# AdaptiveCity/deepdish

Measured on AMD Instinct MI355X. Metric: end-to-end frames/sec (detect+encode+track) at 640x480, higher is better.
Workload: dtype i8 (reference: uint8); encoder f16; 1 GPU; SSD-MobileNet-v1 uint8-quantised (300x300) + MARS-64x32x3 + deep_sort on synthetic 640x480 BGR frames, ~20 synthetic detections/frame (BASELINE.json configs[1]); streams_per_gpu=3072, worker_threads_per_gpu=2, parallelism=independent streams, 3072 per GPU in 2 worker groups, weights=seeded synthetic (seed 1234)

## Files before the change

### deepdish_amd/csrc/cost_dev.h

```cpp
#pragma once
#include <hip/hip_runtime.h>

namespace costdev {

typedef float f32x4 __attribute__((ext_vector_type(4)));

__device__ __forceinline__ double iou_tlwh(const double *a, const double *b) {
    const double ax2 = a[0] + a[2], ay2 = a[1] + a[3];
    const double bx2 = b[0] + b[2], by2 = b[1] + b[3];
    const double tlx = fmax(a[0], b[0]), tly = fmax(a[1], b[1]);
    const double brx = fmin(ax2, bx2), bry = fmin(ay2, by2);
    const double w = fmax(0.0, brx - tlx), h = fmax(0.0, bry - tly);
    const double inter = w * h;
    const double area_a = a[2] * a[3];
    const double area_b = b[2] * b[3];
    return inter / (area_a + area_b - inter);
}

constexpr int GAL_CH_SHIFT = 5, GAL_CH = 1 << GAL_CH_SHIFT;
constexpr int GAL_ARENA_SHIFT = 12, GAL_ARENA_CHUNKS = 1 << GAL_ARENA_SHIFT;

__device__ __forceinline__ float *gal_row(float *const *arenas, int chunk, int off) {
    return arenas[chunk >> GAL_ARENA_SHIFT] + ((size_t)(chunk & (GAL_ARENA_CHUNKS - 1)) * GAL_CH + off) * 128;
}

struct FlatRows {
    const float *base;
    __device__ __forceinline__ const float *row(int r) const { return base + (size_t)r * 128; }
};

struct ChunkRows {
    float *const *arenas;
    const int *tab;
    __device__ __forceinline__ const float *row(int r) const { return gal_row(arenas, tab[r >> GAL_CH_SHIFT], r & (GAL_CH - 1)); }
};

template <class Rows>
__device__ __forceinline__ float nn_max_dot(const Rows rows, int count,
                                            const float *__restrict__ feats, int d0, int n_d, int lane) {
    const int c = lane & 15, q = lane >> 4;
    const int dd = min(d0 + c, n_d - 1);
    f32x4 b[8];
    const float *fp = feats + (size_t)dd * 128 + 4 * q;
#pragma unroll
    for (int s = 0; s < 8; ++s) b[s] = *reinterpret_cast<const f32x4 *>(fp + 16 * s);
    float best = -__builtin_inff();
    for (int g = 0; g < count; g += 16) {
        const int r = min(g + c, count - 1);
        const float *ap = rows.row(r) + 4 * q;
        f32x4 acc = {0.f, 0.f, 0.f, 0.f};
#pragma unroll
        for (int s = 0; s < 8; ++s) {
            const f32x4 a = *reinterpret_cast<const f32x4 *>(ap + 16 * s);
#pragma unroll
            for (int j = 0; j < 4; ++j) acc = __builtin_amdgcn_mfma_f32_16x16x4f32(a[j], b[s][j], acc, 0, 0, 0);
        }
        best = fmaxf(best, fmaxf(fmaxf(acc[0], acc[1]), fmaxf(acc[2], acc[3])));
    }
    best = fmaxf(best, __shfl_xor(best, 16, 64));
    best = fmaxf(best, __shfl_xor(best, 32, 64));
    return best;
}

template <class Rows>
__device__ __forceinline__ float nn_min_sqdist(const Rows rows, int count,
                                               const float *__restrict__ feats, int d0, int n_d, int lane) {
    const int c = lane & 15, q = lane >> 4;
    const int dd = min(d0 + c, n_d - 1);
    f32x4 b[8];
    const float *fp = feats + (size_t)dd * 128 + 4 * q;
    f32x4 b2 = {0.f, 0.f, 0.f, 0.f};
#pragma unroll
    for (int s = 0; s < 8; ++s) {
        b[s] = *reinterpret_cast<const f32x4 *>(fp + 16 * s);
        b2 += b[s] * b[s];
    }
    float qn = (b2[0] + b2[1]) + (b2[2] + b2[3]);
    qn += __shfl_xor(qn, 16, 64);
    qn += __shfl_xor(qn, 32, 64);
    float best = __builtin_inff();
    for (int g = 0; g < count; g += 16) {
        const int r = min(g + c, count - 1);
        const float *ap = rows.row(r) + 4 * q;
        f32x4 acc = {0.f, 0.f, 0.f, 0.f}, a2 = {0.f, 0.f, 0.f, 0.f};
#pragma unroll
        for (int s = 0; s < 8; ++s) {
            const f32x4 a = *reinterpret_cast<const f32x4 *>(ap + 16 * s);
            a2 += a * a;
#pragma unroll
            for (int j = 0; j < 4; ++j) acc = __builtin_amdgcn_mfma_f32_16x16x4f32(a[j], b[s][j], acc, 0, 0, 0);
        }
        float rn = (a2[0] + a2[1]) + (a2[2] + a2[3]);
        rn += __shfl_xor(rn, 16, 64);
        rn += __shfl_xor(rn, 32, 64);
#pragma unroll
        for (int j = 0; j < 4; ++j) {
            const float gn = __shfl(rn, 4 * q + j, 64);
            best = fminf(best, fmaxf(0.f, (-2.f * acc[j] + gn) + qn));
        }
    }
    best = fminf(best, __shfl_xor(best, 16, 64));
    best = fminf(best, __shfl_xor(best, 32, 64));
    return best;
}

}
```

### deepdish_amd/csrc/tracker.hip

```cpp
#include <algorithm>
#include <atomic>
#include <numeric>
#include "common.h"
#include "hostpool.h"
#include "kalman_dev.h"
#include "cost_dev.h"

namespace {
using namespace kfdev;
using namespace costdev;

constexpr double GATE_4DOF = 9.4877;
constexpr double INFTY_COST = 1e5;
enum { TENTATIVE = 1, CONFIRMED = 2, DELETED = 3 };
enum { METRIC_COSINE = 0, METRIC_EUCLIDEAN = 1 };
enum { ASSOC_HOST = 0, ASSOC_DEVICE = 1 };

__device__ __forceinline__ void tlwh_to_xyah(const double *b, double z[4]) {
    z[0] = b[0] + b[2] / 2;
    z[1] = b[1] + b[3] / 2;
    z[2] = b[2] / b[3];
    z[3] = b[3];
}

template <int Metric>
__global__ __launch_bounds__(256) void tracker_assoc_k(
    const double *__restrict__ means, const double *__restrict__ covs, float *const *__restrict__ arenas,
    const int *__restrict__ tab, int tab_stride, const int *__restrict__ row_slot, const int *__restrict__ row_state,
    const int *__restrict__ row_tsu, const int *__restrict__ row_det_off, const int *__restrict__ row_ndet,
    const int *__restrict__ row_cost_off, const int *__restrict__ row_iou_delta, const int *__restrict__ row_gcount,
    const double *__restrict__ det_tlwh, const float *__restrict__ feats_n, double *__restrict__ cost) {
    const int row = blockIdx.x;
    const int wave = threadIdx.x >> 6, lane = threadIdx.x & 63;
    const int n_det = row_ndet[row];
    const int d0 = blockIdx.y * 64 + wave * 16;
    if (d0 >= n_det) return;
    const int slot = row_slot[row];
    const int det_off = row_det_off[row];
    const bool confirmed = row_state[row] == CONFIRMED;
    float best = 0.f;
    if (confirmed) {
        if constexpr (Metric == METRIC_EUCLIDEAN)
            best = nn_min_sqdist(ChunkRows{arenas, tab + (size_t)slot * tab_stride}, row_gcount[row],
                                 feats_n + (size_t)det_off * 128, d0, n_det, lane);
        else
            best = nn_max_dot(ChunkRows{arenas, tab + (size_t)slot * tab_stride}, row_gcount[row],
                              feats_n + (size_t)det_off * 128, d0, n_det, lane);
    }
    const int d = d0 + (lane & 15);
    if ((lane >> 4) != 0 || d >= n_det) return;
    const double *m = means + (size_t)slot * 8;
    const double *b = det_tlwh + (size_t)(det_off + d) * 4;
    const size_t o = (size_t)row_cost_off[row] + d;
    if (confirmed) {
        double S[16], z[4];
        innovation_cov(covs + (size_t)slot * 64, m[3], S);
        const Chol4 c = chol4(S);
        tlwh_to_xyah(b, z);
        const double mm[4] = {m[0], m[1], m[2], m[3]};
        const double d2 = maha2(c, mm, z, 0);
        if constexpr (Metric == METRIC_EUCLIDEAN) cost[o] = d2 > GATE_4DOF ? INFTY_COST : (double)best;
        else cost[o] = d2 > GATE_4DOF ? INFTY_COST : (double)(1.0f - best);
    }
    double ci = INFTY_COST;
    if (row_tsu[row] <= 1) {
        double t[4];
        t[3] = m[3];
        t[2] = m[2] * m[3];
        t[0] = m[0] - t[2] / 2;
        t[1] = m[1] - t[3] / 2;
        ci = 1.0 - iou_tlwh(t, b);
    }
    cost[o + row_iou_delta[row]] = ci;
}

__global__ __launch_bounds__(256) void tracker_apply_k(
    double *__restrict__ means, double *__restrict__ covs, float *const *__restrict__ arenas,
    const int *__restrict__ pair_slot, const int *__restrict__ pair_det, const int *__restrict__ pair_row, int n_upd,
    int n_new, const double *__restrict__ det_tlwh, const float *__restrict__ feats_n) {
    const int w = (blockIdx.x * blockDim.x + threadIdx.x) >> 6;
    const int lane = threadIdx.x & 63;
    if (w >= n_upd + n_new) return;
    const int slot = pair_slot[w], det = pair_det[w], grow = pair_row[w];
    double z[4];
    tlwh_to_xyah(det_tlwh + (size_t)det * 4, z);
    double *P = covs + (size_t)slot * 64, *m = means + (size_t)slot * 8;
    if (w < n_upd) update_wave(P, m, z, lane);
    else initiate_wave(P, m, z, lane);
    const float2 f = reinterpret_cast<const float2 *>(feats_n + (size_t)det * 128)[lane];
    reinterpret_cast<float2 *>(gal_row(arenas, grow >> GAL_CH_SHIFT, grow & (GAL_CH - 1)))[lane] = f;
}

__global__ void tab_scatter_k(int *__restrict__ tab, const int *__restrict__ upd, int n) {
    const int i = blockIdx.x * blockDim.x + threadIdx.x;
    if (i < n) tab[upd[2 * i]] = upd[2 * i + 1];
}

struct TrackRec {
    int64_t id;
    int state, tsu, hits, age, slot, last_det;
};

}

constexpr int GAL_MAX_ARENAS = 4096;
struct TrackerPool {
    dd_ctx *ctx = nullptr;
    int slots = 0, refs = 0;
    int metric = 0;
    double *d_means = nullptr, *d_covs = nullptr;
    std::vector<float *> arenas;
    float **d_arenas = nullptr;
    std::vector<int> free_chunks;
    std::vector<std::vector<int>> slot_chunks;
    std::vector<int> slot_total;
    int *d_tab = nullptr, tab_stride = 0;
    std::vector<int> tab_upd;
    int tab_need = 0;
    DevBuf d_tabupd;
    PinBuf h_tabupd;
    DevBuf d_pred, d_in, d_feats_raw, d_feats_n, d_cost, d_pairs, d_gather, d_assoc;
    PinBuf h_pred, h_in, h_cost, h_pairs, h_gather, h_assoc;
    bool pred_inflight = false;
    int assoc = 0;
    bool upd_inflight = false;
    bool dev_decided = false;
    bool cost_on_host = false;
    std::vector<int> assoc_base;
    long long n_dev_updates = 0, n_host_updates = 0, n_fallback_streams = 0;
    long long assoc_d2h_bytes = 0;
    long long n_stream_param_launches = 0;
    std::vector<dd_tracker *> cur;
    std::vector<int> det_off, cost_base;
    int D = 0, R = 0, ng = 0;
    bool have_cost = false;
};

struct dd_tracker {
    TrackerPool *pool = nullptr;
    int slot_base = 0;
    double max_cos = 0.2, max_iou = 0.7;
    int max_age = 30, n_init = 3, budget = 0, tcap = 0;
    std::vector<TrackRec> tracks, deleted;
    std::vector<int> free_slots, pending_free;
    std::vector<double> live_means, dead_means;
    std::vector<int> last_pairs;
    int64_t next_id = 1;
    int ph_n = 0, ph_T = 0, ph_cost_base = -1;
    std::vector<int> m_upd, m_new;
};

namespace {

void min_cost_matching(const double *full, int n_det, double max_distance, const std::vector<int> &rows,
                       const std::vector<int> &dets, std::vector<std::pair<int, int>> &matches,
                       std::vector<int> &un_rows, std::vector<int> &un_dets) {
    un_rows.clear();
    un_dets.clear();
    if (rows.empty() || dets.empty()) {
        un_rows = rows;
        un_dets = dets;
        return;
    }
    const int nr = (int)rows.size(), nc = (int)dets.size();
    std::vector<double> c((size_t)nr * nc);
    for (int r = 0; r < nr; ++r)
        for (int q = 0; q < nc; ++q) {
            const double v = full[(size_t)rows[r] * n_det + dets[q]];
            c[(size_t)r * nc + q] = v > max_distance ? max_distance + 1e-5 : v;
        }
    std::vector<int> ri(std::min(nr, nc)), ci(std::min(nr, nc));
    const int np = ddk::lsap(c.data(), nr, nc, ri.data(), ci.data());
    std::vector<char> row_used(nr, 0), col_used(nc, 0);
    for (int p = 0; p < np; ++p) { row_used[ri[p]] = 1; col_used[ci[p]] = 1; }
    for (int q = 0; q < nc; ++q) if (!col_used[q]) un_dets.push_back(dets[q]);
    for (int r = 0; r < nr; ++r) if (!row_used[r]) un_rows.push_back(rows[r]);
    for (int p = 0; p < np; ++p) {
        if (c[(size_t)ri[p] * nc + ci[p]] > max_distance) {
            un_rows.push_back(rows[ri[p]]);
            un_dets.push_back(dets[ci[p]]);
        } else {
            matches.emplace_back(rows[ri[p]], dets[ci[p]]);
        }
    }
}

int pool_create(dd_ctx *ctx, int slots, int gallery_rows_hint, TrackerPool **out) {
    TrackerPool *p = new TrackerPool();
    p->ctx = ctx; p->slots = slots;
    DD_HIP(hipSetDevice(ctx->device));
    DD_HIP(hipMalloc(&p->d_means, (size_t)slots * 8 * sizeof(double)));
    DD_HIP(hipMalloc(&p->d_covs, (size_t)slots * 64 * sizeof(double)));
    DD_HIP(hipMalloc(&p->d_arenas, (size_t)GAL_MAX_ARENAS * sizeof(float *)));
    DD_HIP(hipMemset(p->d_arenas, 0, (size_t)GAL_MAX_ARENAS * sizeof(float *)));
    p->tab_stride = std::max(1, dd_ceil_div(gallery_rows_hint, GAL_CH));
    DD_HIP(hipMalloc(&p->d_tab, (size_t)slots * p->tab_stride * sizeof(int)));
    DD_HIP(hipMemset(p->d_tab, 0, (size_t)slots * p->tab_stride * sizeof(int)));
    p->slot_chunks.resize(slots);
    p->slot_total.assign(slots, 0);
    *out = p;
    return DD_OK;
}

int pool_add_arena(TrackerPool *p) {
    DD_REQUIRE((int)p->arenas.size() < GAL_MAX_ARENAS, DD_E_CAPACITY, "tracker gallery: %d arenas of 64 MiB exhausted", GAL_MAX_ARENAS);
    float *a = nullptr;
    const hipError_t e = hipMalloc(&a, (size_t)GAL_ARENA_CHUNKS * GAL_CH * 128 * sizeof(float));
    if (e != hipSuccess) {
        (void)hipGetLastError();
        dd_set_error("tracker gallery: device memory exhausted after %zu arenas of 64 MiB (%s); nn_budget bounds a gallery",
                     p->arenas.size(), hipGetErrorString(e));
        return DD_E_CAPACITY;
    }
    const int k = (int)p->arenas.size();
    p->arenas.push_back(a);
    DD_HIP(hipMemcpy(p->d_arenas + k, &a, sizeof(float *), hipMemcpyHostToDevice));
    for (int c = GAL_ARENA_CHUNKS - 1; c >= 0; --c) p->free_chunks.push_back(k * GAL_ARENA_CHUNKS + c);
    return DD_OK;
}

int gallery_place(TrackerPool *p, int slot, int budget, int *row_out) {
    const int total = p->slot_total[slot];
    const int pos = budget > 0 ? total % budget : total;
    const int ci = pos >> GAL_CH_SHIFT;
    std::vector<int> &chs = p->slot_chunks[slot];
    if (ci >= (int)chs.size()) {
        p->tab_need = std::max(p->tab_need, ci + 1);
        if (p->free_chunks.empty()) {
            const int rc = pool_add_arena(p);
            if (rc != DD_OK) return rc;
        }
        const int c = p->free_chunks.back();
        p->free_chunks.pop_back();
        chs.push_back(c);
        p->tab_upd.push_back(slot);
        p->tab_upd.push_back(ci);
        p->tab_upd.push_back(c);
    }
    *row_out = chs[ci] * GAL_CH + (pos & (GAL_CH - 1));
    p->slot_total[slot] = total + 1;
    return DD_OK;
}

inline int gallery_count(const TrackerPool *p, int slot, int budget) {
    const int total = p->slot_total[slot];
    return budget > 0 ? std::min(total, budget) : total;
}

void gallery_free_slot(TrackerPool *p, int slot) {
    for (int c : p->slot_chunks[slot]) p->free_chunks.push_back(c);
    p->slot_chunks[slot].clear();
    p->slot_total[slot] = 0;
}

int gallery_flush(TrackerPool *p, hipStream_t s) {
    if (p->tab_need > p->tab_stride) {
        int stride = p->tab_stride;
        while (p->tab_need > stride) stride *= 2;
        DD_HIP(hipStreamSynchronize(s));
        const size_t n = (size_t)p->slots * stride;
        int *fresh = nullptr;
        DD_HIP(hipMalloc(&fresh, n * sizeof(int)));
        std::vector<int> host(n, 0);
        for (int sl = 0; sl < p->slots; ++sl)
            for (size_t i = 0; i < p->slot_chunks[sl].size(); ++i) host[(size_t)sl * stride + i] = p->slot_chunks[sl][i];
        const hipError_t e = hipMemcpy(fresh, host.data(), n * sizeof(int), hipMemcpyHostToDevice);
        if (e != hipSuccess) { (void)hipFree(fresh); DD_HIP(e); }
        (void)hipFree(p->d_tab);
        p->d_tab = fresh; p->tab_stride = stride;
        p->tab_upd.clear();
        return DD_OK;
    }
    const int n = (int)p->tab_upd.size() / 3;
    if (n == 0) return DD_OK;
    int rc;
    if ((rc = p->h_tabupd.reserve((size_t)n * 2 * sizeof(int))) != DD_OK) return rc;
    if ((rc = p->d_tabupd.reserve((size_t)n * 2 * sizeof(int))) != DD_OK) return rc;
    int *h = p->h_tabupd.as<int>();
    for (int i = 0; i < n; ++i) {
        h[2 * i] = p->tab_upd[3 * i] * p->tab_stride + p->tab_upd[3 * i + 1];
        h[2 * i + 1] = p->tab_upd[3 * i + 2];
    }
    p->tab_upd.clear();
    DD_HIP(hipMemcpyAsync(p->d_tabupd.p, h, (size_t)n * 2 * sizeof(int), hipMemcpyHostToDevice, s));
    hipLaunchKernelGGL(tab_scatter_k, dim3(dd_ceil_div(n, 256)), dim3(256), 0, s, p->d_tab, p->d_tabupd.as<int>(), n);
    DD_LAUNCH_CHECK();
    return DD_OK;
}

void pool_release(TrackerPool *p) {
    if (!p || --p->refs > 0) return;
    (void)hipFree(p->d_means); (void)hipFree(p->d_covs);
    for (float *a : p->arenas) (void)hipFree(a);
    (void)hipFree(p->d_arenas); (void)hipFree(p->d_tab);
    for (DevBuf *b : {&p->d_pred, &p->d_in, &p->d_feats_raw, &p->d_feats_n, &p->d_cost, &p->d_pairs, &p->d_gather, &p->d_tabupd, &p->d_assoc}) b->release();
    for (PinBuf *b : {&p->h_pred, &p->h_in, &p->h_cost, &p->h_pairs, &p->h_gather, &p->h_tabupd, &p->h_assoc}) b->release();
    delete p;
}

dd_tracker *tracker_new(TrackerPool *pool, int slot_base, int tcap, double max_cos, double max_iou, int max_age, int n_init,
                        int budget) {
    dd_tracker *t = new dd_tracker();
    t->pool = pool; pool->refs += 1;
    t->slot_base = slot_base; t->tcap = tcap;
    t->max_cos = max_cos; t->max_iou = max_iou; t->max_age = max_age; t->n_init = n_init;
    t->budget = budget > 0 ? budget : 0;
    t->free_slots.resize(tcap);
    for (int i = 0; i < tcap; ++i) t->free_slots[i] = slot_base + tcap - 1 - i;
    return t;
}

}

namespace ddk {

int tracker_group_create(dd_ctx *ctx, int n, double max_cos, double max_iou, int max_age, int n_init, int budget, int tcap,
                         int gcap, dd_tracker **out) {
    TrackerPool *pool = nullptr;
    int rc = pool_create(ctx, n * tcap, gcap, &pool);
    if (rc != DD_OK) return rc;
    for (int i = 0; i < n; ++i) out[i] = tracker_new(pool, i * tcap, tcap, max_cos, max_iou, max_age, n_init, budget);
    return DD_OK;
}

int tracker_set_params(dd_tracker *t, const double *max_cos, const double *max_iou, const int *max_age, const int *n_init) {
    DD_REQUIRE(t, DD_E_ARG, "tracker_set_params: NULL tracker");
    DD_REQUIRE(!t->pool->upd_inflight, DD_E_STATE, "tracker parameters: an update of the group is in flight");
    if (max_cos) t->max_cos = *max_cos;
    if (max_iou) t->max_iou = *max_iou;
    if (max_age) t->max_age = *max_age;
    if (n_init) t->n_init = *n_init;
    return DD_OK;
}

int tracker_reset(dd_tracker *t) {
    DD_REQUIRE(t, DD_E_ARG, "tracker_reset: NULL tracker");
    TrackerPool *p = t->pool;
    DD_REQUIRE(!p->upd_inflight, DD_E_STATE, "tracker reset: an update of the group is in flight");
    for (int sl : t->pending_free) gallery_free_slot(p, sl);
    for (auto &tr : t->tracks) gallery_free_slot(p, tr.slot);
    t->pending_free.clear(); t->tracks.clear(); t->deleted.clear();
    t->live_means.clear(); t->dead_means.clear(); t->last_pairs.clear(); t->m_upd.clear(); t->m_new.clear();
    t->next_id = 1;
    t->ph_n = t->ph_T = 0; t->ph_cost_base = -1;
    t->free_slots.resize(t->tcap);
    for (int i = 0; i < t->tcap; ++i) t->free_slots[i] = t->slot_base + t->tcap - 1 - i;
    return DD_OK;
}

long long tracker_group_stream_param_launches(const dd_tracker *any) { return any ? any->pool->n_stream_param_launches : 0; }

int tracker_group_set_metric(dd_tracker *any, int metric) {
    DD_REQUIRE(any && (metric == METRIC_COSINE || metric == METRIC_EUCLIDEAN), DD_E_ARG,
               "tracker metric must be 0 (cosine) or 1 (euclidean), got %d", metric);
    TrackerPool *p = any->pool;
    DD_REQUIRE(p->arenas.empty() || p->metric == metric, DD_E_STATE, "tracker metric: the group already holds gallery rows");
    p->metric = metric;
    return DD_OK;
}

int tracker_group_set_association(dd_tracker *any, int where) {
    DD_REQUIRE(any && (where == ASSOC_HOST || where == ASSOC_DEVICE), DD_E_ARG,
               "tracker association must be 0 (host) or 1 (device), got %d", where);
    DD_REQUIRE(!any->pool->upd_inflight, DD_E_STATE, "tracker association: an update of the group is in flight");
    any->pool->assoc = where;
    return DD_OK;
}

int trackers_predict(dd_tracker **ts, int S) {
    if (S <= 0) return DD_OK;
    TrackerPool *p = ts[0]->pool;
    hipStream_t s = p->ctx->stream;
    int n = 0;
    for (int z = 0; z < S; ++z) {
        dd_tracker *t = ts[z];
        for (int sl : t->pending_free) { gallery_free_slot(p, sl); t->free_slots.push_back(sl); }
        t->pending_free.clear();
        n += (int)t->tracks.size();
    }
    if (n == 0) return DD_OK;
    int rc;
    if (p->pred_inflight) DD_HIP(hipStreamSynchronize(s));
    p->pred_inflight = true;
    if ((rc = p->h_pred.reserve((size_t)n * sizeof(int))) != DD_OK) return rc;
    if ((rc = p->d_pred.reserve((size_t)n * sizeof(int))) != DD_OK) return rc;
    int *h = p->h_pred.as<int>();
    int k = 0;
    for (int z = 0; z < S; ++z)
        for (auto &tr : ts[z]->tracks) {
            h[k++] = tr.slot;
            tr.age += 1;
            tr.tsu += 1;
        }
    DD_HIP(hipMemcpyAsync(p->d_pred.p, h, (size_t)n * sizeof(int), hipMemcpyHostToDevice, s));
    return ddk::kf_predict(s, p->d_means, p->d_covs, p->d_pred.as<int>(), n);
}

int trackers_update_begin(dd_tracker **ts, int S, const double *tlwh_host, const float *feats, int feats_on_device,
                          const int *det_off) {
    TrackerPool *p = ts[0]->pool;
    hipStream_t s = p->ctx->stream;
    int rc;
    if ((p->tab_need > p->tab_stride || !p->tab_upd.empty()) && (rc = gallery_flush(p, s)) != DD_OK) return rc;
    p->cur.assign(ts, ts + S);
    p->det_off.assign(det_off, det_off + S + 1);
    p->cost_base.assign(S, 0);
    const int D = det_off[S];
    int R = 0, maxn = 0;
    size_t cost_total = 0;
    for (int z = 0; z < S; ++z) {
        dd_tracker *t = ts[z];
        t->last_pairs.clear();
        for (auto &tr : t->tracks) tr.last_det = -1;
        t->ph_n = det_off[z + 1] - det_off[z];
        t->ph_T = (int)t->tracks.size();
        p->cost_base[z] = (int)cost_total;
        cost_total += (size_t)2 * t->ph_T * t->ph_n;
        R += t->ph_T;
        maxn = std::max(maxn, t->ph_n);
    }
    p->D = D; p->R = R; p->have_cost = false;
    bool use_dev = p->assoc == ASSOC_DEVICE;
    for (int z = 0; z < S && use_dev; ++z) use_dev = ts[z]->ph_T <= DD_ASSOC_DEVICE_MAX && ts[z]->ph_n <= DD_ASSOC_DEVICE_MAX;
    p->dev_decided = use_dev; p->cost_on_host = false;
    p->assoc_base.assign(S, -1);
    long long &n_updates = use_dev ? p->n_dev_updates : p->n_host_updates;
    if (D == 0) {
        n_updates += 1;
        p->upd_inflight = true;
        return DD_OK;
    }
    bool par_differ = false;
    for (int z = 1; z < S && use_dev && !par_differ; ++z)
        par_differ = ts[z]->max_cos != ts[0]->max_cos || ts[z]->max_iou != ts[0]->max_iou || ts[z]->max_age != ts[0]->max_age;
    const size_t off_rows = (size_t)D * 4 * sizeof(double);
    const size_t off_desc = off_rows + (size_t)8 * R * sizeof(int);
    const size_t off_par = (off_desc + (size_t)5 * S * sizeof(int) + 7) / 8 * 8, off_age = off_par + (size_t)2 * S * sizeof(double);
    const size_t in_bytes = !use_dev ? off_desc : par_differ ? off_age + (size_t)S * sizeof(int) : off_desc + (size_t)5 * S * sizeof(int);
    if ((rc = p->h_in.reserve(in_bytes + 64)) != DD_OK) return rc;
    if ((rc = p->d_in.reserve(in_bytes + 64)) != DD_OK) return rc;
    char *h = p->h_in.as<char>();
    memcpy(h, tlwh_host, (size_t)D * 4 * sizeof(double));
    int *hr = reinterpret_cast<int *>(h + off_rows);
    int *h_slot = hr, *h_state = hr + R, *h_tsu = hr + 2 * R, *h_doff = hr + 3 * R, *h_nd = hr + 4 * R, *h_coff = hr + 5 * R,
        *h_idel = hr + 6 * R, *h_gcnt = hr + 7 * R;
    int r = 0;
    for (int z = 0; z < S; ++z) {
        dd_tracker *t = ts[z];
        for (int i = 0; i < t->ph_T; ++i, ++r) {
            h_slot[r] = t->tracks[i].slot;
            h_state[r] = t->tracks[i].state;
            h_tsu[r] = t->tracks[i].tsu;
            h_doff[r] = det_off[z];
            h_nd[r] = t->ph_n;
            h_coff[r] = p->cost_base[z] + i * t->ph_n;
            h_idel[r] = t->ph_T * t->ph_n;
            h_gcnt[r] = gallery_count(p, t->tracks[i].slot, t->budget);
        }
    }
    int n_dec = 0;
    size_t out_ints = 0;
    if (use_dev) {
        int *hd = reinterpret_cast<int *>(h + off_desc);
        double *hpd = reinterpret_cast<double *>(h + off_par);
        int *hpa = reinterpret_cast<int *>(h + off_age);
        int row_base = 0;
        for (int z = 0; z < S; ++z) {
            const dd_tracker *t = ts[z];
            if (t->ph_T > 0 && t->ph_n > 0) {
                if (par_differ) { hpd[2 * n_dec] = t->max_cos; hpd[2 * n_dec + 1] = t->max_iou; hpa[n_dec] = t->max_age; }
                int *e = hd + 5 * n_dec++;
                e[0] = row_base; e[1] = t->ph_T; e[2] = t->ph_n; e[3] = p->cost_base[z]; e[4] = (int)out_ints;
                p->assoc_base[z] = (int)out_ints;
                out_ints += ddk::assoc_out_ints(t->ph_T, t->ph_n);
            }
            row_base += t->ph_T;
        }
    }
    char *d = p->d_in.as<char>();
    DD_HIP(hipMemcpyAsync(d, h, in_bytes, hipMemcpyHostToDevice, s));
    const bool euclid = p->metric == METRIC_EUCLIDEAN;
    if ((rc = p->d_feats_n.reserve((size_t)D * 128 * sizeof(float))) != DD_OK) return rc;
    if (euclid) {
        DD_HIP(hipMemcpyAsync(p->d_feats_n.p, feats, (size_t)D * 128 * sizeof(float),
                              feats_on_device ? hipMemcpyDeviceToDevice : hipMemcpyHostToDevice, s));
    } else {
        const float *raw = feats;
        if (!feats_on_device) {
            if ((rc = p->d_feats_raw.reserve((size_t)D * 128 * sizeof(float))) != DD_OK) return rc;
            DD_HIP(hipMemcpyAsync(p->d_feats_raw.p, feats, (size_t)D * 128 * sizeof(float), hipMemcpyHostToDevice, s));
            raw = p->d_feats_raw.as<float>();
        }
        if ((rc = ddk::normalize_rows(s, raw, p->d_feats_n.as<float>(), D)) != DD_OK) return rc;
    }
    if (R > 0 && cost_total > 0) {
        if ((rc = p->d_cost.reserve(cost_total * sizeof(double))) != DD_OK) return rc;
        if (!use_dev && (rc = p->h_cost.reserve(cost_total * sizeof(double))) != DD_OK) return rc;
        const int *dr = reinterpret_cast<const int *>(d + off_rows);
        hipLaunchKernelGGL(euclid ? tracker_assoc_k<METRIC_EUCLIDEAN> : tracker_assoc_k<METRIC_COSINE>, dim3(R, dd_ceil_div(maxn, 64)),
                           dim3(256), 0, s, p->d_means, p->d_covs,
                           p->d_arenas, p->d_tab, p->tab_stride, dr, dr + R, dr + 2 * R, dr + 3 * R, dr + 4 * R, dr + 5 * R,
                           dr + 6 * R, dr + 7 * R, reinterpret_cast<const double *>(d), p->d_feats_n.as<float>(),
                           p->d_cost.as<double>());
        DD_LAUNCH_CHECK();
        if (use_dev) {
            if ((rc = p->d_assoc.reserve(out_ints * sizeof(int))) != DD_OK) return rc;
            if ((rc = p->h_assoc.reserve(out_ints * sizeof(int))) != DD_OK) return rc;
            if (par_differ) {
                if ((rc = ddk::assoc_match_streams(s, p->d_cost.as<double>(), dr + R, dr + 2 * R, reinterpret_cast<const int *>(d + off_desc), n_dec,
                                                   reinterpret_cast<const double *>(d + off_par), reinterpret_cast<const int *>(d + off_age),
                                                   p->d_assoc.as<int>())) != DD_OK) return rc;
                p->n_stream_param_launches += n_dec > 0;
            } else
            if ((rc = ddk::assoc_match(s, p->d_cost.as<double>(), dr + R, dr + 2 * R, reinterpret_cast<const int *>(d + off_desc), n_dec,
                                       ts[0]->max_cos, ts[0]->max_iou, ts[0]->max_age, p->d_assoc.as<int>())) != DD_OK) return rc;
            DD_HIP(hipMemcpyAsync(p->h_assoc.p, p->d_assoc.p, out_ints * sizeof(int), hipMemcpyDeviceToHost, s));
            p->assoc_d2h_bytes += (long long)(out_ints * sizeof(int));
        } else {
            DD_HIP(hipMemcpyAsync(p->h_cost.p, p->d_cost.p, cost_total * sizeof(double), hipMemcpyDeviceToHost, s));
            p->cost_on_host = true;
            p->assoc_d2h_bytes += (long long)(cost_total * sizeof(double));
        }
        p->have_cost = true;
    }
    n_updates += 1;
    p->upd_inflight = true;
    return DD_OK;
}

namespace {
int match_one_stream(TrackerPool *p, dd_tracker *t, int z) {
    const int n = t->ph_n, T = t->ph_T, doff = p->det_off[z];
    std::vector<int> matches, un_rows_final, un_dets;
    t->m_upd.clear(); t->m_new.clear();
    t->ph_cost_base = (n > 0 && T > 0 && p->have_cost) ? p->cost_base[z] : -1;
    const int *dev = (p->dev_decided && n > 0 && T > 0 && p->assoc_base[z] >= 0) ? p->h_assoc.as<int>() + p->assoc_base[z] : nullptr;
    if (dev && dev[0] == 0) {
        const int *pm = dev + 4, *pr = pm + 2 * std::min(T, n), *pd = pr + T;
        matches.assign(pm, pm + 2 * dev[1]);
        un_rows_final.assign(pr, pr + dev[2]);
        un_dets.assign(pd, pd + dev[3]);
    } else {
        std::vector<int> state(T), tsu(T);
        for (int i = 0; i < T; ++i) { state[i] = t->tracks[i].state; tsu[i] = t->tracks[i].tsu; }
        const double *app = (n > 0 && T > 0) ? p->h_cost.as<double>() + p->cost_base[z] : nullptr;
        ddk::match_decide_host(app, app ? app + (size_t)T * n : nullptr, T, n, state.data(), tsu.data(), t->max_cos, t->max_iou, t->max_age,
                               matches, un_rows_final, un_dets);
    }
    for (size_t k = 0; k + 1 < matches.size(); k += 2) {
        const int row = matches[k], det = matches[k + 1];
        TrackRec &tr = t->tracks[row];
        tr.hits += 1;
        tr.tsu = 0;
        tr.last_det = det;
        if (tr.state == TENTATIVE && tr.hits >= t->n_init) tr.state = CONFIRMED;
        t->m_upd.push_back(tr.slot); t->m_upd.push_back(doff + det);
        t->last_pairs.push_back(row);
        t->last_pairs.push_back(det);
    }
    for (int r : un_rows_final) {
        TrackRec &tr = t->tracks[r];
        if (tr.state == TENTATIVE) tr.state = DELETED;
        else if (tr.tsu > t->max_age) tr.state = DELETED;
    }
    DD_REQUIRE((int)t->free_slots.size() >= (int)un_dets.size(), DD_E_CAPACITY,
               "dd_tracker_update: track capacity %d exhausted", t->tcap);
    for (int dd : un_dets) {
        TrackRec tr;
        tr.id = t->next_id++;
        tr.state = TENTATIVE; tr.tsu = 0; tr.hits = 1; tr.age = 1;
        tr.slot = t->free_slots.back();
        t->free_slots.pop_back();
        tr.last_det = dd;
        t->tracks.push_back(tr);
        t->m_new.push_back(tr.slot); t->m_new.push_back(doff + dd);
    }
    std::vector<TrackRec> live;
    t->deleted.clear();
    for (auto &tr : t->tracks) (tr.state == DELETED ? t->deleted : live).push_back(tr);
    t->tracks.swap(live);
    for (auto &tr : t->deleted) t->pending_free.push_back(tr.slot);
    return DD_OK;
}
}

void match_decide_host(const double *app, const double *iou, int T, int n, const int *state, const int *tsu, double max_cos,
                       double max_iou, int max_age, std::vector<int> &matches_flat, std::vector<int> &un_rows_final, std::vector<int> &un_dets) {
    std::vector<std::pair<int, int>> matches;
    std::vector<int> lvl_rows, tmp_rows, tmp_dets, confirmed, unconfirmed;
    matches_flat.clear(); un_rows_final.clear(); un_dets.clear();
    if (n > 0 && T > 0) {
        for (int i = 0; i < T; ++i) (state[i] == CONFIRMED ? confirmed : unconfirmed).push_back(i);
        un_dets.resize(n);
        std::iota(un_dets.begin(), un_dets.end(), 0);
        for (int level = 0; level < max_age; ++level) {
            if (un_dets.empty()) break;
            lvl_rows.clear();
            for (int k : confirmed) if (tsu[k] == 1 + level) lvl_rows.push_back(k);
            if (lvl_rows.empty()) continue;
            min_cost_matching(app, n, max_cos, lvl_rows, un_dets, matches, tmp_rows, tmp_dets);
            un_dets = tmp_dets;
        }
        std::vector<int> matched_rows, un_a_all;
        for (auto &m : matches) matched_rows.push_back(m.first);
        ddk::pyset_difference_order(confirmed, matched_rows, un_a_all);
        std::vector<int> iou_rows = unconfirmed, un_rows_a;
        for (int k : un_a_all) {
            if (tsu[k] == 1) iou_rows.push_back(k); else un_rows_a.push_back(k);
        }
        std::vector<int> un_rows_b;
        min_cost_matching(iou, n, max_iou, iou_rows, un_dets, matches, un_rows_b, tmp_dets);
        un_dets = tmp_dets;
        un_rows_final = un_rows_a;
        un_rows_final.insert(un_rows_final.end(), un_rows_b.begin(), un_rows_b.end());
    } else {
        un_dets.resize(n);
        std::iota(un_dets.begin(), un_dets.end(), 0);
        for (int i = 0; i < T; ++i) un_rows_final.push_back(i);
    }
    for (auto &m : matches) { matches_flat.push_back(m.first); matches_flat.push_back(m.second); }
}

namespace {
int update_match(dd_tracker **ts, int S) {
    TrackerPool *p = ts[0]->pool;
    hipStream_t s = p->ctx->stream;
    p->pred_inflight = false;
    int rc;
    const int D = p->D;
    if (p->dev_decided && p->have_cost) {
        size_t total = 0;
        for (int z = 0; z < S; ++z) total += (size_t)2 * ts[z]->ph_T * ts[z]->ph_n;
        int n_back = 0;
        for (int z = 0; z < S; ++z) {
            if (p->assoc_base[z] < 0 || p->h_assoc.as<int>()[p->assoc_base[z]] == 0) continue;
            if (n_back++ == 0 && (rc = p->h_cost.reserve(total * sizeof(double))) != DD_OK) return rc;
            const size_t bytes = (size_t)2 * ts[z]->ph_T * ts[z]->ph_n * sizeof(double);
            DD_HIP(hipMemcpyAsync(p->h_cost.as<double>() + p->cost_base[z], p->d_cost.as<double>() + p->cost_base[z], bytes,
                                  hipMemcpyDeviceToHost, s));
            p->assoc_d2h_bytes += (long long)bytes;
        }
        if (n_back) DD_HIP(hipStreamSynchronize(s));
        p->n_fallback_streams += n_back;
    }
    size_t max_pairs = (size_t)p->R + D;
    if ((rc = p->h_pairs.reserve(max_pairs * 3 * sizeof(int) + 64)) != DD_OK) return rc;
    if ((rc = p->d_pairs.reserve(max_pairs * 3 * sizeof(int) + 64)) != DD_OK) return rc;
    std::vector<int> upd_slot, upd_det, upd_row, new_slot, new_det, new_row;
    std::atomic<int> first_err{DD_OK};
    ddk::parallel_for(S, 8, [&](int z0, int z1) {
        for (int z = z0; z < z1; ++z) {
            const int r = match_one_stream(p, ts[z], z);
            if (r != DD_OK) { int ok = DD_OK; first_err.compare_exchange_strong(ok, r); }
        }
    });
    if (first_err.load() != DD_OK) {
        int zbad = -1;
        for (int z = 0; z < S && zbad < 0; ++z) if (ts[z]->free_slots.empty()) zbad = z;
        dd_set_error("dd_tracker_update: track capacity %d exhausted (stream %d of %d in the group); the group's state is no longer consistent: "
                     "recreate it with a larger track_capacity", zbad >= 0 ? ts[zbad]->tcap : ts[0]->tcap, zbad, S);
        return first_err.load();
    }
    for (int z = 0; z < S; ++z) {
        dd_tracker *t = ts[z];
        for (size_t i = 0; i + 1 < t->m_upd.size(); i += 2) {
            int grow = 0;
            if ((rc = gallery_place(p, t->m_upd[i], t->budget, &grow)) != DD_OK) return rc;
            upd_slot.push_back(t->m_upd[i]); upd_det.push_back(t->m_upd[i + 1]); upd_row.push_back(grow);
        }
        for (size_t i = 0; i + 1 < t->m_new.size(); i += 2) {
            int grow = 0;
            if ((rc = gallery_place(p, t->m_new[i], t->budget, &grow)) != DD_OK) return rc;
            new_slot.push_back(t->m_new[i]); new_det.push_back(t->m_new[i + 1]); new_row.push_back(grow);
        }
    }
    const int n_upd = (int)upd_slot.size(), n_new = (int)new_slot.size(), np = n_upd + n_new;
    if (np > 0) {
        int *hp = p->h_pairs.as<int>();
        for (int i = 0; i < n_upd; ++i) { hp[i] = upd_slot[i]; hp[np + i] = upd_det[i]; hp[2 * np + i] = upd_row[i]; }
        for (int i = 0; i < n_new; ++i) { hp[n_upd + i] = new_slot[i]; hp[np + n_upd + i] = new_det[i]; hp[2 * np + n_upd + i] = new_row[i]; }
        int *dp = p->d_pairs.as<int>();
        DD_HIP(hipMemcpyAsync(dp, hp, (size_t)3 * np * sizeof(int), hipMemcpyHostToDevice, s));
        hipLaunchKernelGGL(tracker_apply_k, dim3(dd_ceil_div(np, 4)), dim3(256), 0, s, p->d_means, p->d_covs, p->d_arenas,
                           dp, dp + np, dp + 2 * np, n_upd, n_new, p->d_in.as<double>(), p->d_feats_n.as<float>());
        DD_LAUNCH_CHECK();
    }
    if ((rc = gallery_flush(p, s)) != DD_OK) return rc;
    int ng = 0;
    for (int z = 0; z < S; ++z) ng += (int)(ts[z]->tracks.size() + ts[z]->deleted.size());
    p->ng = ng;
    if (ng > 0) {
        if ((rc = p->h_gather.reserve((size_t)ng * (sizeof(int) + 8 * sizeof(double)))) != DD_OK) return rc;
        if ((rc = p->d_gather.reserve((size_t)ng * (sizeof(int) + 8 * sizeof(double)))) != DD_OK) return rc;
        double *hg = p->h_gather.as<double>();
        int *hs = reinterpret_cast<int *>(hg + (size_t)ng * 8);
        int k = 0;
        for (int z = 0; z < S; ++z) {
            for (auto &tr : ts[z]->tracks) hs[k++] = tr.slot;
            for (auto &tr : ts[z]->deleted) hs[k++] = tr.slot;
        }
        double *dg = p->d_gather.as<double>();
        int *ds = reinterpret_cast<int *>(dg + (size_t)ng * 8);
        DD_HIP(hipMemcpyAsync(ds, hs, (size_t)ng * sizeof(int), hipMemcpyHostToDevice, s));
        if ((rc = ddk::gather_state(s, p->d_means, p->d_covs, ds, ng, dg, nullptr)) != DD_OK) return rc;
        DD_HIP(hipMemcpyAsync(hg, dg, (size_t)ng * 8 * sizeof(double), hipMemcpyDeviceToHost, s));
    }
    return DD_OK;
}
}

int trackers_update_match(dd_tracker **ts, int S) {
    const int rc = update_match(ts, S);
    if (rc != DD_OK) ts[0]->pool->upd_inflight = false;
    return rc;
}

int trackers_update_end(dd_tracker **ts, int S) {
    TrackerPool *p = ts[0]->pool;
    p->upd_inflight = false;
    const double *hg = p->h_gather.as<double>();
    size_t k = 0;
    for (int z = 0; z < S; ++z) {
        dd_tracker *t = ts[z];
        const size_t nl = t->tracks.size(), nd = t->deleted.size();
        t->live_means.assign(hg + k * 8, hg + (k + nl) * 8);
        k += nl;
        t->dead_means.assign(hg + k * 8, hg + (k + nd) * 8);
        k += nd;
    }
    return DD_OK;
}

int tracker_read_host(dd_tracker *t, int which, int64_t *ints6_host, double *means_host) {
    const std::vector<TrackRec> &v = which == 0 ? t->tracks : t->deleted;
    const std::vector<double> &mm = which == 0 ? t->live_means : t->dead_means;
    const int n = (int)v.size();
    if (ints6_host)
        for (int i = 0; i < n; ++i) {
            int64_t *o = ints6_host + (size_t)i * 6;
            o[0] = v[i].id; o[1] = v[i].state; o[2] = v[i].tsu; o[3] = v[i].hits; o[4] = v[i].age; o[5] = v[i].last_det;
        }
    if (means_host && n) {
        DD_REQUIRE(mm.size() == (size_t)n * 8, DD_E_STATE, "dd_tracker_read: means are only mirrored after update()");
        memcpy(means_host, mm.data(), (size_t)n * 8 * sizeof(double));
    }
    return DD_OK;
}


void tracker_pool_view(dd_tracker *t, TrackerPoolView *v) {
    TrackerPool *p = t->pool;
    v->d_arenas = p->d_arenas; v->d_means = p->d_means; v->d_covs = p->d_covs;
    v->arena_shift = GAL_ARENA_SHIFT; v->metric = p->metric; v->budget = t->budget; v->tcap = t->tcap;
    v->max_cos = t->max_cos; v->max_iou = t->max_iou; v->max_age = t->max_age; v->n_init = t->n_init;
    v->upd_inflight = p->upd_inflight;
}

int tracker_export(dd_tracker *t, int64_t *next_id, std::vector<TrackView> &live, std::vector<TrackView> &dead) {
    TrackerPool *p = t->pool;
    DD_REQUIRE(t->live_means.size() == t->tracks.size() * 8 && t->dead_means.size() == t->deleted.size() * 8, DD_E_STATE,
               "snapshot: the tracker's means are not mirrored (between a per-track call and the next update)");
    *next_id = t->next_id;
    for (int which = 0; which < 2; ++which) {
        const std::vector<TrackRec> &v = which == 0 ? t->tracks : t->deleted;
        std::vector<TrackView> &out = which == 0 ? live : dead;
        out.clear();
        for (const TrackRec &tr : v) {
            TrackView w;
            w.id = tr.id; w.state = tr.state; w.tsu = tr.tsu; w.hits = tr.hits; w.age = tr.age; w.last_det = tr.last_det; w.slot = tr.slot;
            w.slot_total = p->slot_total[tr.slot];
            w.n_rows = gallery_count(p, tr.slot, t->budget);
            w.chunks = p->slot_chunks[tr.slot].data();
            w.n_chunks = dd_ceil_div(w.n_rows, GAL_CH);
            DD_REQUIRE(w.n_chunks <= (int)p->slot_chunks[tr.slot].size(), DD_E_STATE, "snapshot: track %lld has %d rows in %zu chunks", (long long)tr.id,
                       w.n_rows, p->slot_chunks[tr.slot].size());
            out.push_back(w);
        }
    }
    return DD_OK;
}

int tracker_pool_reserve_chunks(dd_tracker *any, size_t n) {
    TrackerPool *p = any->pool;
    while (p->free_chunks.size() < n) {
        const int rc = pool_add_arena(p);
        if (rc != DD_OK) return rc;
    }
    return DD_OK;
}

int tracker_import(dd_tracker *t, int64_t next_id, const TrackLoad *tr_in, int n_live, int n_dead, std::vector<int> &slots_out,
                   std::vector<int> &chunks_out) {
    TrackerPool *p = t->pool;
    DD_REQUIRE(n_live >= 0 && n_dead >= 0 && n_live + n_dead <= t->tcap, DD_E_CAPACITY, "restore: %d tracks, track_capacity %d", n_live + n_dead, t->tcap);
    int rc = tracker_reset(t);
    if (rc != DD_OK) return rc;
    size_t need = 0;
    for (int i = 0; i < n_live + n_dead; ++i) need += (size_t)dd_ceil_div(tr_in[i].n_rows, GAL_CH);
    DD_REQUIRE(p->free_chunks.size() >= need, DD_E_STATE, "restore: %zu gallery chunks were not reserved", need);
    t->next_id = next_id;
    t->live_means.resize((size_t)n_live * 8); t->dead_means.resize((size_t)n_dead * 8);
    for (int i = 0; i < n_live + n_dead; ++i) {
        const TrackLoad &in = tr_in[i];
// ... 299 lines not shown
```

Baseline: 146,100 frames/s.

## Gate-first association: compute appearance distance only for gated detections

The association kernel now runs as one wave per row and detection block. It computes the Mahalanobis gate and IoU costs first, then ballots and compacts the detections that pass the gate, and runs the gallery nearest-neighbour MFMA loop only for those. The gallery walk loads each chunk base pointer once instead of doing a table lookup per row, and the single-tile path software-pipelines the row fetches using sched barriers. This is meant to cut wasted MFMA work and gallery loads for detections that are gated out. In exchange it adds compaction overhead and gives up the previous parallelism of four waves per block.

```diff
diff --git a/deepdish_amd/csrc/cost_dev.h b/deepdish_amd/csrc/cost_dev.h
--- a/deepdish_amd/csrc/cost_dev.h
+++ b/deepdish_amd/csrc/cost_dev.h
@@ -4,6 +4,7 @@
 namespace costdev {
 
 typedef float f32x4 __attribute__((ext_vector_type(4)));
+typedef __attribute__((address_space(1))) f32x4 global_f32x4;
 
 __device__ __forceinline__ double iou_tlwh(const double *a, const double *b) {
     const double ax2 = a[0] + a[2], ay2 = a[1] + a[3];
@@ -29,11 +30,127 @@
     __device__ __forceinline__ const float *row(int r) const { return base + (size_t)r * 128; }
 };
 
-struct ChunkRows {
+struct ChunkWalk {
     float *const *arenas;
     const int *tab;
-    __device__ __forceinline__ const float *row(int r) const { return gal_row(arenas, tab[r >> GAL_CH_SHIFT], r & (GAL_CH - 1)); }
+    int count;
+    const float *cur, *nxt;
+    __device__ __forceinline__ const float *base(int ch) const { return gal_row(arenas, tab[ch], 0); }
+    __device__ __forceinline__ ChunkWalk(float *const *arenas_, const int *tab_, int count_) : arenas(arenas_), tab(tab_), count(count_) {
+        cur = nxt = nullptr;
+        if (count > 0) cur = nxt = base(0);
+        if (count > GAL_CH) nxt = base(1);
+    }
+    __device__ __forceinline__ void fetch(f32x4 a[8], int g, int lane) {
+        if (g > 0 && (g & (GAL_CH - 1)) == 0) {
+            cur = nxt;
+            if (g + GAL_CH < count) nxt = base((g >> GAL_CH_SHIFT) + 1);
+        }
+        const int r = min(g + (lane & 15), count - 1);
+        const global_f32x4 *ap = (const global_f32x4 *)(cur + (size_t)(r & (GAL_CH - 1)) * 128 + 4 * (lane >> 4));
+#pragma unroll
+        for (int s = 0; s < 8; ++s) a[s] = ap[4 * s];
+    }
 };
+
+__device__ __forceinline__ float det_frag(f32x4 b[8], const float *__restrict__ feats, int dd, int lane) {
+    const float *fp = feats + (size_t)dd * 128 + 4 * (lane >> 4);
+    f32x4 b2 = {0.f, 0.f, 0.f, 0.f};
+#pragma unroll
+    for (int s = 0; s < 8; ++s) {
+        b[s] = *reinterpret_cast<const f32x4 *>(fp + 16 * s);
+        b2 += b[s] * b[s];
+    }
+    float qn = (b2[0] + b2[1]) + (b2[2] + b2[3]);
+    qn += __shfl_xor(qn, 16, 64);
+    qn += __shfl_xor(qn, 32, 64);
+    return qn;
+}
+
+template <bool Euclid>
+__device__ __forceinline__ float tile_best(const f32x4 a[8], const f32x4 b[8], float qn, float best, int lane) {
+    f32x4 acc = {0.f, 0.f, 0.f, 0.f}, a2 = {0.f, 0.f, 0.f, 0.f};
+#pragma unroll
+    for (int s = 0; s < 8; ++s) {
+        if constexpr (Euclid) a2 += a[s] * a[s];
+#pragma unroll
+        for (int j = 0; j < 4; ++j) acc = __builtin_amdgcn_mfma_f32_16x16x4f32(a[s][j], b[s][j], acc, 0, 0, 0);
+    }
+    if constexpr (!Euclid) {
+        return fmaxf(best, fmaxf(fmaxf(acc[0], acc[1]), fmaxf(acc[2], acc[3])));
+    } else {
+        const int q = lane >> 4;
+        float rn = (a2[0] + a2[1]) + (a2[2] + a2[3]);
+        rn += __shfl_xor(rn, 16, 64);
+        rn += __shfl_xor(rn, 32, 64);
+#pragma unroll
+        for (int j = 0; j < 4; ++j) {
+            const float gn = __shfl(rn, 4 * q + j, 64);
+            best = fminf(best, fmaxf(0.f, (-2.f * acc[j] + gn) + qn));
+        }
+        return best;
+    }
+}
+
+template <bool Euclid>
+__device__ __forceinline__ float best_across_q(float best) {
+    if constexpr (Euclid) {
+        best = fminf(best, __shfl_xor(best, 16, 64));
+        return fminf(best, __shfl_xor(best, 32, 64));
+    } else {
+        best = fmaxf(best, __shfl_xor(best, 16, 64));
+        return fmaxf(best, __shfl_xor(best, 32, 64));
+    }
+}
+
+template <bool Euclid>
+__device__ __forceinline__ float nn_one_tile(ChunkWalk w, const float *__restrict__ feats, int dd, int lane) {
+    f32x4 b[8], a[8], an[8];
+    const float qn = det_frag(b, feats, dd, lane);
+    float best = Euclid ? __builtin_inff() : -__builtin_inff();
+    if (w.count > 0) {
+        w.fetch(a, 0, lane);
+        int g = 16;
+        for (; g + 16 < w.count; g += 32) {
+            w.fetch(an, g, lane);
+            __builtin_amdgcn_sched_barrier(0);
+            best = tile_best<Euclid>(a, b, qn, best, lane);
+            __builtin_amdgcn_sched_barrier(0);
+            w.fetch(a, g + 16, lane);
+            __builtin_amdgcn_sched_barrier(0);
+            best = tile_best<Euclid>(an, b, qn, best, lane);
+            __builtin_amdgcn_sched_barrier(0);
+        }
+        if (g < w.count) {
+            w.fetch(an, g, lane);
+            __builtin_amdgcn_sched_barrier(0);
+            best = tile_best<Euclid>(a, b, qn, best, lane);
+            best = tile_best<Euclid>(an, b, qn, best, lane);
+        } else {
+            best = tile_best<Euclid>(a, b, qn, best, lane);
+        }
+    }
+    return best_across_q<Euclid>(best);
+}
+
+template <bool Euclid>
+__device__ __forceinline__ void nn_many_tiles(ChunkWalk w, const float *__restrict__ feats, const int dd[4], int n_tiles, int lane, float best[4]) {
+#pragma unroll
+    for (int t = 0; t < 4; ++t) best[t] = Euclid ? __builtin_inff() : -__builtin_inff();
+    for (int g = 0; g < w.count; g += 16) {
+        f32x4 a[8];
+        w.fetch(a, g, lane);
+#pragma unroll
+        for (int t = 0; t < 4; ++t)
+            if (t < n_tiles) {
+                f32x4 b[8];
+                const float qn = det_frag(b, feats, dd[t], lane);
+                best[t] = tile_best<Euclid>(a, b, qn, best[t], lane);
+            }
+    }
+#pragma unroll
+    for (int t = 0; t < 4; ++t) best[t] = best_across_q<Euclid>(best[t]);
+}
 
 template <class Rows>
 __device__ __forceinline__ float nn_max_dot(const Rows rows, int count,
diff --git a/deepdish_amd/csrc/tracker.hip b/deepdish_amd/csrc/tracker.hip
--- a/deepdish_amd/csrc/tracker.hip
+++ b/deepdish_amd/csrc/tracker.hip
@@ -24,54 +24,77 @@
 }
 
 template <int Metric>
-__global__ __launch_bounds__(256) void tracker_assoc_k(
+__global__ __launch_bounds__(64) void tracker_assoc_k(
     const double *__restrict__ means, const double *__restrict__ covs, float *const *__restrict__ arenas,
     const int *__restrict__ tab, int tab_stride, const int *__restrict__ row_slot, const int *__restrict__ row_state,
     const int *__restrict__ row_tsu, const int *__restrict__ row_det_off, const int *__restrict__ row_ndet,
     const int *__restrict__ row_cost_off, const int *__restrict__ row_iou_delta, const int *__restrict__ row_gcount,
     const double *__restrict__ det_tlwh, const float *__restrict__ feats_n, double *__restrict__ cost) {
-    const int row = blockIdx.x;
-    const int wave = threadIdx.x >> 6, lane = threadIdx.x & 63;
+    constexpr bool Euclid = Metric == METRIC_EUCLIDEAN;
+    __shared__ int sel[64];
+    const int row = blockIdx.x, lane = threadIdx.x;
     const int n_det = row_ndet[row];
-    const int d0 = blockIdx.y * 64 + wave * 16;
-    if (d0 >= n_det) return;
+    const int d_base = blockIdx.y * 64;
+    if (d_base >= n_det) return;
     const int slot = row_slot[row];
     const int det_off = row_det_off[row];
     const bool confirmed = row_state[row] == CONFIRMED;
-    float best = 0.f;
-    if (confirmed) {
-        if constexpr (Metric == METRIC_EUCLIDEAN)
-            best = nn_min_sqdist(ChunkRows{arenas, tab + (size_t)slot * tab_stride}, row_gcount[row],
-                                 feats_n + (size_t)det_off * 128, d0, n_det, lane);
-        else
-            best = nn_max_dot(ChunkRows{arenas, tab + (size_t)slot * tab_stride}, row_gcount[row],
-                              feats_n + (size_t)det_off * 128, d0, n_det, lane);
-    }
-    const int d = d0 + (lane & 15);
-    if ((lane >> 4) != 0 || d >= n_det) return;
-    const double *m = means + (size_t)slot * 8;
-    const double *b = det_tlwh + (size_t)(det_off + d) * 4;
+    const int d = d_base + lane;
+    const bool valid = d < n_det;
     const size_t o = (size_t)row_cost_off[row] + d;
-    if (confirmed) {
-        double S[16], z[4];
-        innovation_cov(covs + (size_t)slot * 64, m[3], S);
-        const Chol4 c = chol4(S);
-        tlwh_to_xyah(b, z);
-        const double mm[4] = {m[0], m[1], m[2], m[3]};
-        const double d2 = maha2(c, mm, z, 0);
-        if constexpr (Metric == METRIC_EUCLIDEAN) cost[o] = d2 > GATE_4DOF ? INFTY_COST : (double)best;
-        else cost[o] = d2 > GATE_4DOF ? INFTY_COST : (double)(1.0f - best);
-    }
-    double ci = INFTY_COST;
-    if (row_tsu[row] <= 1) {
-        double t[4];
-        t[3] = m[3];
-        t[2] = m[2] * m[3];
-        t[0] = m[0] - t[2] / 2;
-        t[1] = m[1] - t[3] / 2;
-        ci = 1.0 - iou_tlwh(t, b);
-    }
-    cost[o + row_iou_delta[row]] = ci;
+    bool inside = false;
+    if (valid) {
+        const double *m = means + (size_t)slot * 8;
+        const double *b = det_tlwh + (size_t)(det_off + d) * 4;
+        if (confirmed) {
+            double S[16], z[4];
+            innovation_cov(covs + (size_t)slot * 64, m[3], S);
+            const Chol4 c = chol4(S);
+            tlwh_to_xyah(b, z);
+            const double mm[4] = {m[0], m[1], m[2], m[3]};
+            const double d2 = maha2(c, mm, z, 0);
+            inside = !(d2 > GATE_4DOF);
+            if (!inside) cost[o] = INFTY_COST;
+        }
+        double ci = INFTY_COST;
+        if (row_tsu[row] <= 1) {
+            double t[4];
+            t[3] = m[3];
+            t[2] = m[2] * m[3];
+            t[0] = m[0] - t[2] / 2;
+            t[1] = m[1] - t[3] / 2;
+            ci = 1.0 - iou_tlwh(t, b);
+        }
+        cost[o + row_iou_delta[row]] = ci;
+    }
+    const unsigned long long gate = __ballot(inside);
+    if (gate == 0) return;
+    const int n_in = __popcll(gate);
+    const int p = __popcll(gate & ((1ull << lane) - 1));
+    if (inside) sel[p] = lane;
+    __syncthreads();
+    const float *feats = feats_n + (size_t)(det_off + d_base) * 128;
+    ChunkWalk walk(arenas, tab + (size_t)slot * tab_stride, row_gcount[row]);
+    const int c = lane & 15;
+    float best;
+    if (n_in <= 16) {
+        const float b0 = nn_one_tile<Euclid>(walk, feats, sel[min(c, n_in - 1)], lane);
+        best = __shfl(b0, p & 15, 64);
+    } else {
+        const int n_tiles = (n_in + 15) >> 4;
+        int dd[4];
+        float bt[4];
+#pragma unroll
+        for (int t = 0; t < 4; ++t) dd[t] = sel[min(16 * t + c, n_in - 1)];
+        nn_many_tiles<Euclid>(walk, feats, dd, n_tiles, lane, bt);
+        best = 0.f;
+#pragma unroll
+        for (int t = 0; t < 4; ++t) {
+            const float v = __shfl(bt[t], p & 15, 64);
+            if ((p >> 4) == t) best = v;
+        }
+    }
+    if (inside) cost[o] = Euclid ? (double)best : (double)(1.0f - best);
 }
 
 __global__ __launch_bounds__(256) void tracker_apply_k(
@@ -498,7 +521,7 @@
         if (!use_dev && (rc = p->h_cost.reserve(cost_total * sizeof(double))) != DD_OK) return rc;
         const int *dr = reinterpret_cast<const int *>(d + off_rows);
         hipLaunchKernelGGL(euclid ? tracker_assoc_k<METRIC_EUCLIDEAN> : tracker_assoc_k<METRIC_COSINE>, dim3(R, dd_ceil_div(maxn, 64)),
-                           dim3(256), 0, s, p->d_means, p->d_covs,
+                           dim3(64), 0, s, p->d_means, p->d_covs,
                            p->d_arenas, p->d_tab, p->tab_stride, dr, dr + R, dr + 2 * R, dr + 3 * R, dr + 4 * R, dr + 5 * R,
                            dr + 6 * R, dr + 7 * R, reinterpret_cast<const double *>(d), p->d_feats_n.as<float>(),
                            p->d_cost.as<double>());
```

New measurement: 145,400 frames/s. Within noise of the previous version (-0.5%).
